# dask-contrib/dask-sql

Measured on NVIDIA H100. Metric: rows/s on Q3-shaped filter->join->groupby, higher is better.
Workload: dtype f64

## Files before the change

### dask-sql_b200/_lib.py

```python
import ctypes as C
import os

HERE = os.path.dirname(os.path.abspath(__file__))
LIB_PATH = os.environ.get("B200SQL_LIB") or os.path.join(HERE, "libb200sql.so")

I64, F64, U8 = 0, 1, 2
U32 = 3
COL_SENTINEL = 1
MAX_COLS, MAX_TERMS, MAX_AGGS, MAX_KEYS, MAX_GATHER, MAX_PROG = 16, 8, 8, 4, 8, 64
TILE = 4096
EQ, NE, LT, LE, GT, GE, IS_NULL, IS_NOT_NULL, IS_TRUE = range(9)
AGG_SUM, AGG_SUMF, AGG_MIN, AGG_MAX, AGG_COUNT, AGG_AND, AGG_OR, AGG_XOR = range(8)
JOIN_INNER, JOIN_LEFT, JOIN_SEMI, JOIN_ANTI = range(4)
EMPTY_KEY = -(1 << 63)

OP_LOAD, OP_CONST_I, OP_CONST_F, OP_CONST_NULL, OP_I2F, OP_F2I = 0, 1, 2, 3, 4, 5
OP_ADD_I, OP_SUB_I, OP_MUL_I, OP_DIV_I, OP_NEG_I, OP_ABS_I, OP_MOD_I = 10, 11, 12, 13, 14, 15, 16
OP_ADD_F, OP_SUB_F, OP_MUL_F, OP_DIV_F, OP_NEG_F, OP_ABS_F, OP_SQRT_F = 20, 21, 22, 23, 24, 25, 26
OP_EQ_I, OP_EQ_F = 30, 40
OP_AND, OP_OR, OP_NOT, OP_ISNULL_I, OP_ISNULL_F, OP_CASE, OP_FILLNA, OP_ORD2F = 50, 51, 52, 53, 54, 55, 56, 57
OP_DATEPART, OP_ADDMONTHS, OP_MAP = 60, 61, 62
OP_MATH_F, OP_MATH2_F, OP_POW_I = 63, 64, 65
(FN_CEIL, FN_FLOOR, FN_TRUNC, FN_ROUND, FN_SIGN, FN_DEGREES, FN_RADIANS, FN_EXP, FN_LN, FN_LOG10, FN_CBRT, FN_SIN,
 FN_COS, FN_TAN, FN_COT, FN_ASIN, FN_ACOS, FN_ATAN, FN_ATAN2, FN_POW, FN_MOD) = range(21)
# ... 149 lines not shown
    "b2_join_onepass": [C.POINTER(Scan), C.POINTER(C.c_int32), C.POINTER(JoinTable), C.c_int32, C.c_int32, _P, C.c_int32,
                        C.POINTER(C.c_int32), C.POINTER(_P), C.POINTER(_P), C.c_int32, C.POINTER(Col),
                        C.POINTER(C.c_int64), C.POINTER(_P), C.POINTER(_P), _P],
    "b2_join_agg": [C.POINTER(Scan), C.c_int32, C.POINTER(JoinTable), C.c_int32, C.POINTER(Col), C.POINTER(C.c_int64),
                    C.POINTER(JoinAgg), C.c_int32, _P, _P, C.c_int32, _P, _P],
    "b2_range_partition_hist": [C.POINTER(Scan), C.c_int32, C.c_int64, C.c_int64, C.c_int32, C.c_int32, _P, _P],
    "b2_range_partition_scan": [C.c_int32, _P, _P],
    "b2_range_partition_scatter": [C.POINTER(Scan), C.c_int32, C.c_int64, C.c_int64, C.c_int32, C.c_int32, C.c_int32,
                                   C.POINTER(C.c_int32), _P, C.POINTER(_P), _P, _P],
    "b2_range_partition": [C.POINTER(Scan), C.c_int32, C.c_int64, C.c_int64, C.c_int32, C.c_int32, C.c_int32,
                           C.POINTER(C.c_int32), _P, C.POINTER(_P), _P, _P],
    "b2_iota": [_P, C.c_int64, _P],
    "b2_bitwise_combine": [_P, _P, C.c_int64, C.c_int32, _P],
    "b2_peer_merge": [C.POINTER(PeerMerge), _P],
    "b2_sort_by": [C.POINTER(Col), C.c_int64, C.c_int32, C.c_int32, _P, _P, _P],
    "b2_dense_slots": [C.POINTER(Col), C.c_int64, C.c_int64, C.c_int32, _P, _P],
    "b2_star_build_dense": [C.POINTER(Col), _P, C.c_int64, _P, C.c_int64, C.c_int64, _P, _P, _P],
    "b2_star_build_mark": [C.POINTER(Scan), C.c_int32, C.c_int64, C.c_int64, _P, _P, _P],
    "b2_star_build_rank": [_P, C.c_int64, _P],
    "b2_star_build_fill": [C.POINTER(Scan), C.c_int32, C.c_int32, C.c_int64, C.c_int64, C.c_int64, C.c_int32, _P,
                           _P, _P],
    "b2_star_build_fill_packed": [C.POINTER(Scan), C.c_int32, C.c_int32, C.c_int64, C.c_int64, C.c_int64,
                                  C.c_int32, _P, _P, C.c_int32, _P],
    "b2_star_build_hash": [C.POINTER(Col), _P, C.c_int64, _P, _P, _P, C.c_int64, _P, _P],
    "b2_star_agg": [C.POINTER(Scan), C.c_int32, C.POINTER(StarLookup), C.POINTER(Agg), C.c_int32,
                    C.POINTER(AggState), _P],
    "b2_str_like": [_P, _P, C.c_int64, _P, C.c_int64, C.c_uint32, C.c_int32, _P, _P],
    "b2_str_lower_bound": [_P, _P, C.c_int64, _P, _P, C.c_int64, C.c_int32, _P, _P, _P],
}

EXPORTS = sorted(list(_SIGS) + ["b2_last_error", "b2_num_tiles", "b2_stats_ws_bytes", "b2_scan_agg_ws_bytes",
                                "b2_sort_ws_bytes", "b2_join_onepass_ws_bytes", "b2_range_partition_ws_bytes",
                                "b2_f64_to_ordered", "b2_ordered_to_f64"])


call_times = {} if os.environ.get("B200SQL_CALL_TIMES") == "1" else None


def _wrap(name):
    fn = getattr(_lib, name)
    fn.restype = C.c_int32
    fn.argtypes = _SIGS[name]

    if call_times is not None:
        import time

# ... 47 lines not shown
join_write_gather_keyed = _wrap("b2_join_write_gather_keyed")
join_key_layout = _wrap("b2_join_key_layout")
join_onepass = _wrap("b2_join_onepass")
join_onepass_ws_bytes = _lib.b2_join_onepass_ws_bytes
join_agg = _wrap("b2_join_agg")
range_partition = _wrap("b2_range_partition")
range_partition_hist = _wrap("b2_range_partition_hist")
range_partition_scan = _wrap("b2_range_partition_scan")
range_partition_scatter = _wrap("b2_range_partition_scatter")
range_partition_ws_bytes = _lib.b2_range_partition_ws_bytes
iota = _wrap("b2_iota")
bitwise_combine = _wrap("b2_bitwise_combine")
peer_merge = _wrap("b2_peer_merge")
sort_by = _wrap("b2_sort_by")
_lib.b2_sort_ws_bytes.restype = C.c_int64
_lib.b2_sort_ws_bytes.argtypes = [C.c_int64]
sort_ws_bytes = _lib.b2_sort_ws_bytes
dense_slots = _wrap("b2_dense_slots")
star_build_dense = _wrap("b2_star_build_dense")
star_build_mark = _wrap("b2_star_build_mark")
star_build_rank = _wrap("b2_star_build_rank")
star_build_fill = _wrap("b2_star_build_fill")
star_build_fill_packed = _wrap("b2_star_build_fill_packed")
star_build_hash = _wrap("b2_star_build_hash")
star_agg = _wrap("b2_star_agg")
str_like = _wrap("b2_str_like")
str_lower_bound = _wrap("b2_str_lower_bound")
num_tiles = _lib.b2_num_tiles
stats_ws_bytes = _lib.b2_stats_ws_bytes
scan_agg_ws_bytes = _lib.b2_scan_agg_ws_bytes
f64_to_ordered = _lib.b2_f64_to_ordered
ordered_to_f64 = _lib.b2_ordered_to_f64


def has_symbol(name):
    try:
        getattr(_lib, name)
        return True
    except AttributeError:
        return False
```

### dask-sql_b200/csrc/common.cuh

```cuda
#pragma once
#include <cuda_runtime.h>
#include <stdint.h>
#include <stdio.h>
#include <stdarg.h>
#include "b200sql.h"

#define B2_BLOCK 256
#define B2_WARPS (B2_BLOCK / 32)
#define FULL_MASK 0xffffffffu
#define B2_MAX_PARTIALS (132 * 16)

extern thread_local char g_b2_err[512];
static inline int32_t b2_fail(int32_t code, const char* fmt, ...) {
  va_list ap;
  va_start(ap, fmt);
  vsnprintf(g_b2_err, sizeof(g_b2_err), fmt, ap);
  va_end(ap);
  return code;
}
#define B2_CUDA_TRY(expr)                                                              \
  do {                                                                                 \
    cudaError_t e__ = (expr);                                                          \
    if (e__ != cudaSuccess)                                                            \
      return b2_fail(B2_ERR_CUDA, "%s failed: %s (%s:%d)", #expr, cudaGetErrorString(e__), \
// ... 73 lines not shown

__device__ __forceinline__ uint64_t b2_policy_stream() {
  uint64_t p;
  asm("createpolicy.fractional.L2::evict_first.b64 %0, 1.0;" : "=l"(p));
  return p;
}
__device__ __forceinline__ uint64_t b2_policy_keep() {
  uint64_t p;
  asm("createpolicy.fractional.L2::evict_last.b64 %0, 1.0;" : "=l"(p));
  return p;
}
__device__ __forceinline__ int64_t b2_ld_stream(const int64_t* p) {
  int64_t v;
  asm("ld.global.nc.L2::cache_hint.b64 %0, [%1], %2;" : "=l"(v) : "l"(p), "l"(b2_policy_stream()));
  return v;
}
__device__ __forceinline__ int32_t b2_ld_keep_i32(const int32_t* p) {
  int32_t v;
  asm("ld.global.nc.L2::cache_hint.b32 %0, [%1], %2;" : "=r"(v) : "l"(p), "l"(b2_policy_keep()));
  return v;
}
__device__ __forceinline__ void b2_st_stream(int64_t* p, int64_t v) {
  asm volatile("st.global.L2::cache_hint.b64 [%0], %1, %2;" ::"l"(p), "l"(v), "l"(b2_policy_stream()) : "memory");
}
__device__ __forceinline__ int64_t b2_ld_keep_i64(const int64_t* p) {
  int64_t v;
  asm("ld.global.nc.L2::cache_hint.b64 %0, [%1], %2;" : "=l"(v) : "l"(p), "l"(b2_policy_keep()));
  return v;
}
__device__ __forceinline__ int64_t b2_ld_cg_i64(const int64_t* p) {
  return __ldcg(reinterpret_cast<const long long*>(p));
}

__host__ __device__ __forceinline__ int64_t b2_ordered_from_bits(int64_t b) {
  return b ^ ((b >> 63) & 0x7fffffffffffffffLL);
}

__device__ __forceinline__ bool b2_cmp_i(int op, int64_t a, int64_t b) {
  switch (op) {
    case B2_EQ: return a == b;
    case B2_NE: return a != b;
    case B2_LT: return a < b;
    case B2_LE: return a <= b;
    case B2_GT: return a > b;
    default: return a >= b;
  }
// ... 329 lines not shown
```

### dask-sql_b200/csrc/groupby.cuh

```cuda
#pragma once
#include "common.cuh"
#include "pipeline.cuh"
#include "warpagg.cuh"

#define B2_GB_R 8
#define B2_GB_ROWS_PER_BLOCK (B2_BLOCK * B2_GB_R)
#define B2_MAX_PROBE 1024

template <int R, class LD>
__device__ __forceinline__ void b2_dense_slots_of(const b2_scan_t& s, const LD& ld, int key_col, int64_t kmin,
                                                  int64_t nslots, int64_t (&slot)[R]) {
  const b2_col_t& kc = s.cols[key_col];
  bool full;
  const uint32_t bits = b2_eval_terms<R>(s, ld, full);
  int64_t key[R];
  ld.template load<R>(key_col, bits, full, key);
  uint32_t kvalid = bits;
  if (kc.valid) kvalid = b2_valid_bits<R>(kc.valid, ld.row0, bits);
#pragma unroll
  for (int j = 0; j < R; ++j) {
    slot[j] = -1;
    if ((bits >> j) & 1) {
      if (!((kvalid >> j) & 1)) slot[j] = nslots - 1;
      else {
// ... 205 lines not shown
    out[i] = b2_is_null(key, i, raw) ? null_slot : (int32_t)(raw - kmin);
  }
}

__global__ void __launch_bounds__(B2_BLOCK)
b2_star_build_dense_kernel(const __grid_constant__ b2_col_t pk, const int32_t* __restrict__ sel, int64_t n_sel,
                           const int32_t* __restrict__ slot_of_row, int64_t kmin, int64_t range,
                           int32_t* __restrict__ lookup, int32_t* __restrict__ flags) {
  for (int64_t i = (int64_t)blockIdx.x * B2_BLOCK + threadIdx.x; i < n_sel; i += (int64_t)gridDim.x * B2_BLOCK) {
    const int64_t r = sel ? sel[i] : i;
    const int64_t raw = b2_load_raw(pk, r);
    if (b2_is_null(pk, r, raw)) continue;
    const uint64_t d = (uint64_t)raw - (uint64_t)kmin;
    if (d >= (uint64_t)range) continue;
    const int32_t old = atomicExch(lookup + d, slot_of_row[i]);
    if (old != -1) flags[0] = 1;
  }
}

__device__ __forceinline__ uint32_t b2_slot_word(uint32_t pos, int slot_bits) {
  return slot_bits == 16 ? pos >> 2 : __umulhi(pos, 0x55555556u);
}

template <bool FILL>
__global__ void __launch_bounds__(B2_BLOCK)
b2_star_build_scan_kernel(const __grid_constant__ b2_scan_t s, int pk_col, int grp_col, int64_t pk_min,
                          int64_t pk_range, int64_t grp_min, int32_t null_slot, uint64_t* __restrict__ dir,
                          void* __restrict__ slots, int slot_bits, int32_t* __restrict__ flags) {
  const int tile_off = (threadIdx.x >> 5) * (32 * B2_GB_R) + (threadIdx.x & 31);
  const b2_col_t& pc = s.cols[pk_col];
  const b2_col_t& gc = s.cols[grp_col];
  for (int64_t base = (int64_t)blockIdx.x * B2_GB_ROWS_PER_BLOCK; base < s.n;
       base += (int64_t)gridDim.x * B2_GB_ROWS_PER_BLOCK) {
    const b2_gld ld{&s, base + tile_off};
    bool full;
    const uint32_t bits = b2_eval_terms<B2_GB_R>(s, ld, full);
    int64_t pk[B2_GB_R];
    ld.template load<B2_GB_R>(pk_col, bits, full, pk);
    uint32_t live = bits;
    if (pc.valid) live &= b2_valid_bits<B2_GB_R>(pc.valid, ld.row0, bits);
#pragma unroll
    for (int j = 0; j < B2_GB_R; ++j) {
      const uint64_t d = (uint64_t)pk[j] - (uint64_t)pk_min;
      if (!(((live >> j) & 1) && d < (uint64_t)pk_range)) live &= ~(1u << j);
    }
    if (!FILL) {
#pragma unroll
      for (int j = 0; j < B2_GB_R; ++j) {
        if (!((live >> j) & 1)) continue;
        const uint64_t d = (uint64_t)pk[j] - (uint64_t)pk_min;
        const uint32_t b = 1u << (d & 31);
        if (atomicOr(reinterpret_cast<uint32_t*>(dir + (d >> 5)), b) & b) flags[0] = 1;
      }
    } else {
      int64_t grp[B2_GB_R];
      ld.template load<B2_GB_R>(grp_col, live, false, grp);
      uint32_t gnull = 0;
      if (gc.valid) gnull = live & ~b2_valid_bits<B2_GB_R>(gc.valid, ld.row0, live);
      uint32_t pos[B2_GB_R];
      int32_t v[B2_GB_R];
#pragma unroll
      for (int j = 0; j < B2_GB_R; ++j) {
        pos[j] = 0;
        v[j] = 0;
        if (!((live >> j) & 1)) continue;
        const uint64_t d = (uint64_t)pk[j] - (uint64_t)pk_min;
        const uint64_t w = dir[d >> 5];
        pos[j] = (uint32_t)(w >> 32) + __popc((uint32_t)w & ((1u << (d & 31)) - 1));
        v[j] = (gnull >> j) & 1 ? null_slot : (int32_t)(grp[j] - grp_min);
      }
      if (slot_bits == 32 || slot_bits == 16) {
#pragma unroll
        for (int j = 0; j < B2_GB_R; ++j) {
          if (!((live >> j) & 1)) continue;
          if (slot_bits == 32) static_cast<int32_t*>(slots)[pos[j]] = v[j];
          else static_cast<uint16_t*>(slots)[pos[j]] = (uint16_t)v[j];
        }
      } else {
        unsigned long long e[B2_GB_R], old[B2_GB_R];
        uint32_t q[B2_GB_R], sh[B2_GB_R];
#pragma unroll
        for (int j = 0; j < B2_GB_R; ++j) {
          q[j] = b2_slot_word(pos[j], 21);
          sh[j] = (pos[j] - q[j] * 3) * 21;
          e[j] = ((unsigned long long)(uint32_t)v[j] & 0x1FFFFFull) << sh[j];
          old[j] = 0;
        }
        unsigned long long* w = reinterpret_cast<unsigned long long*>(slots);
        for (uint32_t pend = live; pend;) {
          unsigned long long seen[B2_GB_R];
#pragma unroll
          for (int j = 0; j < B2_GB_R; ++j)
            if ((pend >> j) & 1) seen[j] = atomicCAS(w + q[j], old[j], (old[j] & ~(0x1FFFFFull << sh[j])) | e[j]);
#pragma unroll
          for (int j = 0; j < B2_GB_R; ++j) {
            if (!((pend >> j) & 1)) continue;
            if (seen[j] == old[j]) pend &= ~(1u << j);
            else old[j] = seen[j];
          }
        }
      }
    }
  }
}

#define B2_RANK_PER_THREAD 8
#define B2_RANK_TILE (B2_BLOCK * B2_RANK_PER_THREAD)

__device__ __forceinline__ uint32_t* b2_rank_half(uint64_t* dir, int64_t i) {
  return reinterpret_cast<uint32_t*>(dir + i) + 1;
}

template <bool WRITE>
__global__ void __launch_bounds__(B2_BLOCK) b2_star_rank_tile_kernel(uint64_t* __restrict__ dir, int64_t nwords) {
  __shared__ int warp_sums[B2_WARPS];
  __shared__ uint32_t tile_off;
  const int lane = threadIdx.x & 31, warp = threadIdx.x >> 5;
  const int64_t t0 = (int64_t)blockIdx.x * B2_RANK_TILE;
  const int64_t i0 = t0 + (int64_t)threadIdx.x * B2_RANK_PER_THREAD;
  if (WRITE && threadIdx.x == 0) tile_off = *b2_rank_half(dir, t0);
  uint32_t bits[B2_RANK_PER_THREAD];
  int tsum = 0;
#pragma unroll
  for (int k = 0; k < B2_RANK_PER_THREAD; ++k) {
    bits[k] = i0 + k < nwords ? (uint32_t)dir[i0 + k] : 0u;
    tsum += __popc(bits[k]);
  }
  int incl = tsum;
#pragma unroll
  for (int o = 1; o < 32; o <<= 1) {
    const int t = __shfl_up_sync(FULL_MASK, incl, o);
    if (lane >= o) incl += t;
  }
  if (lane == 31) warp_sums[warp] = incl;
  __syncthreads();
  if (!WRITE) {
    if (threadIdx.x == 0) {
      int total = 0;
      for (int w = 0; w < B2_WARPS; ++w) total += warp_sums[w];
      *b2_rank_half(dir, t0) = (uint32_t)total;
    }
    return;
  }
  uint32_t r = tile_off + (uint32_t)(incl - tsum);
  for (int w = 0; w < warp; ++w) r += (uint32_t)warp_sums[w];
#pragma unroll
  for (int k = 0; k < B2_RANK_PER_THREAD; ++k) {
    if (i0 + k < nwords) dir[i0 + k] = (uint64_t)bits[k] | ((uint64_t)r << 32);
    r += __popc(bits[k]);
  }
}

struct b2_scan_io_tile_off {
  uint64_t* dir;
  __device__ int64_t get(int64_t t) const { return *b2_rank_half(dir, t * B2_RANK_TILE); }
  __device__ void put(int64_t t, int64_t v) const { *b2_rank_half(dir, t * B2_RANK_TILE) = (uint32_t)v; }
};

__global__ void __launch_bounds__(B2_SCAN_THREADS) b2_star_rank_carry_kernel(uint64_t* __restrict__ dir, int64_t ntiles) {
  b2_block_exclusive_scan(b2_scan_io_tile_off{dir}, ntiles);
}

__global__ void __launch_bounds__(B2_BLOCK)
b2_star_build_hash_kernel(const __grid_constant__ b2_col_t pk, const int32_t* __restrict__ sel, int64_t n_sel,
                          const int32_t* __restrict__ slot_of_row, int64_t* __restrict__ tk,
                          int32_t* __restrict__ ts, int64_t cap, int32_t* __restrict__ flags) {
  for (int64_t i = (int64_t)blockIdx.x * B2_BLOCK + threadIdx.x; i < n_sel; i += (int64_t)gridDim.x * B2_BLOCK) {
    const int64_t r = sel ? sel[i] : i;
    const int64_t key = b2_load_raw(pk, r);
    if (b2_is_null(pk, r, key)) continue;
    if (key == B2_EMPTY_KEY) { flags[1] = 1; continue; }
    uint64_t h = b2_mix64((uint64_t)key) & (uint64_t)(cap - 1);
// ... 294 lines not shown

int32_t b2_dense_slots(const b2_col_t* key, int64_t n, int64_t kmin, int32_t null_slot, int32_t* out_slot,
                       void* stream) {
  B2_REQUIRE(key && out_slot, "null argument");
  if (n <= 0) return B2_OK;
  int grid = b2_wave_grid(b2_dense_slots_kernel, B2_BLOCK, (n + B2_BLOCK - 1) / B2_BLOCK);
  b2_dense_slots_kernel<<<grid, B2_BLOCK, 0, (cudaStream_t)stream>>>(*key, n, kmin, null_slot, out_slot);
  B2_CHECK_LAUNCH("b2_dense_slots_kernel");
  return B2_OK;
}

int32_t b2_star_build_dense(const b2_col_t* pk, const int32_t* sel, int64_t n_sel, const int32_t* slot_of_row,
                            int64_t kmin, int64_t range, int32_t* lookup, int32_t* d_flags, void* stream) {
  B2_REQUIRE(pk && slot_of_row && lookup && d_flags, "null argument");
  B2_REQUIRE(pk->dtype == B2_I64, "dense lookup needs an int64 key");
  if (n_sel <= 0) return B2_OK;
  int grid = b2_wave_grid(b2_star_build_dense_kernel, B2_BLOCK, (n_sel + B2_BLOCK - 1) / B2_BLOCK);
  b2_star_build_dense_kernel<<<grid, B2_BLOCK, 0, (cudaStream_t)stream>>>(*pk, sel, n_sel, slot_of_row, kmin,
                                                                           range, lookup, d_flags);
  B2_CHECK_LAUNCH("b2_star_build_dense_kernel");
  return B2_OK;
}

static int32_t b2_star_build_pass(bool fill, const b2_scan_t* scan, int32_t pk_col, int32_t grp_col,
                                  int64_t pk_min, int64_t pk_range, int64_t grp_min, int32_t null_slot,
                                  uint64_t* dir, void* slots, int32_t slot_bits, int32_t* d_flags, void* stream) {
  int32_t rc = b2_check_scan(scan);
  if (rc) return rc;
  B2_REQUIRE(pk_col >= 0 && pk_col < scan->ncols && grp_col >= 0 && grp_col < scan->ncols, "column out of range");
  B2_REQUIRE(scan->cols[pk_col].dtype == B2_I64 && scan->cols[grp_col].dtype == B2_I64, "dense keys must be int64");
  B2_REQUIRE(pk_range > 0 && pk_range < ((int64_t)1 << 31), "bad range");
  if (scan->n == 0) return B2_OK;
  int64_t nblk = (scan->n + B2_GB_ROWS_PER_BLOCK - 1) / B2_GB_ROWS_PER_BLOCK;
  if (fill) {
    int grid = b2_wave_grid(b2_star_build_scan_kernel<true>, B2_BLOCK, nblk);
    b2_star_build_scan_kernel<true><<<grid, B2_BLOCK, 0, (cudaStream_t)stream>>>(*scan, pk_col, grp_col, pk_min, pk_range,
                                                                                  grp_min, null_slot, dir, slots, slot_bits, d_flags);
  } else {
    int grid = b2_wave_grid(b2_star_build_scan_kernel<false>, B2_BLOCK, nblk);
    b2_star_build_scan_kernel<false><<<grid, B2_BLOCK, 0, (cudaStream_t)stream>>>(*scan, pk_col, grp_col, pk_min, pk_range,
                                                                                   grp_min, null_slot, dir, slots, slot_bits, d_flags);
  }
  B2_CHECK_LAUNCH("b2_star_build_scan_kernel");
  return B2_OK;
}

int32_t b2_star_build_mark(const b2_scan_t* scan, int32_t pk_col, int64_t pk_min, int64_t pk_range, uint64_t* dir,
                           int32_t* d_flags, void* stream) {
  B2_REQUIRE(dir && d_flags, "null argument");
  return b2_star_build_pass(false, scan, pk_col, pk_col, pk_min, pk_range, 0, 0, dir, nullptr, 32, d_flags, stream);
}

int32_t b2_star_build_rank(uint64_t* dir, int64_t pk_range, void* stream) {
  B2_REQUIRE(dir, "null argument");
  B2_REQUIRE(pk_range > 0 && pk_range < ((int64_t)1 << 31), "bad range");
  const int64_t nwords = (pk_range + 31) / 32;
  const int64_t ntiles = (nwords + B2_RANK_TILE - 1) / B2_RANK_TILE;
  b2_star_rank_tile_kernel<false><<<(unsigned)ntiles, B2_BLOCK, 0, (cudaStream_t)stream>>>(dir, nwords);
  B2_CHECK_LAUNCH("b2_star_rank_tile_kernel<false>");
  b2_star_rank_carry_kernel<<<1, B2_SCAN_THREADS, 0, (cudaStream_t)stream>>>(dir, ntiles);
  B2_CHECK_LAUNCH("b2_star_rank_carry_kernel");
  b2_star_rank_tile_kernel<true><<<(unsigned)ntiles, B2_BLOCK, 0, (cudaStream_t)stream>>>(dir, nwords);
  B2_CHECK_LAUNCH("b2_star_rank_tile_kernel<true>");
  return B2_OK;
}

int32_t b2_star_build_fill(const b2_scan_t* scan, int32_t pk_col, int32_t grp_col, int64_t pk_min,
                           int64_t pk_range, int64_t grp_min, int32_t null_slot, const uint64_t* dir,
                           int32_t* slots, void* stream) {
  return b2_star_build_fill_packed(scan, pk_col, grp_col, pk_min, pk_range, grp_min, null_slot, dir,
                                   reinterpret_cast<uint64_t*>(slots), 32, stream);
}

int32_t b2_star_build_fill_packed(const b2_scan_t* scan, int32_t pk_col, int32_t grp_col, int64_t pk_min,
                                  int64_t pk_range, int64_t grp_min, int32_t null_slot, const uint64_t* dir,
                                  uint64_t* slots, int32_t slot_bits, void* stream) {
  B2_REQUIRE(dir && slots, "null argument");
  B2_REQUIRE(slot_bits == 16 || slot_bits == 21 || slot_bits == 32, "slot_bits must be 16, 21 or 32");
  B2_REQUIRE(slot_bits == 32 || (null_slot >= 0 && null_slot < (1 << slot_bits)), "null_slot does not fit slot_bits");
  B2_REQUIRE(slot_bits == 32 || ((uintptr_t)slots & 7) == 0, "packed slots must be 8-byte aligned");
  return b2_star_build_pass(true, scan, pk_col, grp_col, pk_min, pk_range, grp_min, null_slot,
                            const_cast<uint64_t*>(dir), slots, slot_bits, nullptr, stream);
}

int32_t b2_star_build_hash(const b2_col_t* pk, const int32_t* sel, int64_t n_sel, const int32_t* slot_of_row,
                           int64_t* table_keys, int32_t* table_slots, int64_t cap, int32_t* d_flags,
                           void* stream) {
  B2_REQUIRE(pk && slot_of_row && table_keys && table_slots && d_flags, "null argument");
  B2_REQUIRE(pk->dtype == B2_I64, "star lookup needs an int64 key");
  B2_REQUIRE(b2_pow2(cap), "cap must be a power of two");
  if (n_sel <= 0) return B2_OK;
  int grid = b2_wave_grid(b2_star_build_hash_kernel, B2_BLOCK, (n_sel + B2_BLOCK - 1) / B2_BLOCK);
  b2_star_build_hash_kernel<<<grid, B2_BLOCK, 0, (cudaStream_t)stream>>>(*pk, sel, n_sel, slot_of_row, table_keys,
                                                                          table_slots, cap, d_flags);
  B2_CHECK_LAUNCH("b2_star_build_hash_kernel");
  return B2_OK;
}

int32_t b2_star_agg(const b2_scan_t* scan, int32_t fk_col, const b2_starlookup_t* lk, const b2_agg_t* aggs,
                    int32_t naggs, const b2_aggstate_t* st, void* stream) {
  int32_t rc = b2_check_scan(scan);
  if (rc) return rc;
  b2_aggs_arg aa;
  if ((rc = b2_check_aggs(scan, aggs, naggs, &aa))) return rc;
  if ((rc = b2_check_state(aa, st))) return rc;
// ... 30 lines not shown
```

### dask-sql_b200/executor.py

```python
import ctypes as C
import os
from collections import namedtuple
from typing import Dict, List, Optional, Sequence, Set

import numpy as np
import torch

from . import _lib as L
from . import device as D
from . import expr as E
from . import parallel as P
from . import strings as S
from .device import DeviceColumn, TermSpec, I64, F64, U8
from .expr import Expr, ColRef, Lit, Call
from .frame import LazyFrame, Source, TableSource, JoinSource, AggSource, SortSource, LimitSource
from .table import DeviceTable, HostColumn

DENSE_MAX_SLOTS = 1 << 27
_TORCH_DT = {I64: torch.int64, F64: torch.float64, U8: torch.uint8}

stats = {"launches": 0, "star_fused": 0, "dense_groupby": 0, "hash_groupby": 0, "dense_join": 0,
         "chain_join": 0, "keyed_join": 0, "partitioned_groupby": 0, "h2d_bytes": 0, "d2h_bytes": 0}


# ... 1482 lines not shown
            if part.n == 0:
                continue
            ctx = ScanCtx(part, q.dpred)
            pk_slot, g_slot = ctx.slot(q.pk_e), ctx.slot(q.ge)
            self._only_table_columns(ctx)
            self.dim_launch.append((ctx.scan(), pk_slot, g_slot))
            self.keep.append(ctx)
        self.fact_launch = []
        for part in fparts:
            if part.n == 0:
                continue
            ctx = ScanCtx(part, q.fpred)
            fk_slot = ctx.slot(q.fk_e)
            specs = [(ctx.slot(ka.expr), ka.op) for ka in q.plan.kaggs]
            self._only_table_columns(ctx)
            self.fact_launch.append((ctx.scan(), fk_slot, D.make_aggs(specs), len(specs), part.n))
            self.keep.append(ctx)
        self.slot_bits = _star_slot_bits(self.nslots - 1)
        slots_off, self.flags_off, words = _star_bitmap_words(q.prange, q.dn, self.slot_bits)
        self.lookup = torch.empty(words, dtype=torch.int32, device=dev)
        self.lk = lk = L.StarLookup()
        lk.dense, lk.dir, lk.kmin, lk.range, lk.slot_bits = 2, self.lookup.data_ptr(), q.pmin, q.prange, self.slot_bits
        lk.lookup = self.lookup.data_ptr() + 4 * slots_off
        self.tabs = [GroupState(dev, self.nslots, q.plan, need_present=True,
                                alloc=_padded_slots(self.nslots, q.sharded))]
        self.dirty = [False]
        self.peer = None
        self.epoch = 0
        self.free = [None, None]
        self.merge_bufs = {} if cached else None
        self.runs = 0

    def install_peer_merge(self, state):
        self.tabs, self.dirty, self.peer, self.arena, self.local_ready = state
        stats["peer_merge_plans"] = stats.get("peer_merge_plans", 0) + 1

    def build_peer_merge(self):
        rank, size = P.world()
        dev = self.dev
        alloc = _padded_slots(self.nslots, True)
        proto = self.tabs[0].table
        narr = sum(a is not None for a in proto.acc) + sum(c is not None for c in proto.cnt) + (proto.rows is not None)
        per_table = (narr * alloc * 8 + D.bitmap_words(alloc) * 4) + (narr + 2) * P.PeerArena.ALIGN
        arena = P.PeerArena(2 * per_table + 4 * P.PeerArena.ALIGN, dev)
        _, sig_off = arena.carve(L.MAX_PEERS, torch.int64, 0)
        chunk = alloc // size
# ... 61 lines not shown
            for name in needed:
                c = p[name]
                if not isinstance(c, DeviceColumn):
                    raise _NotPreparable()
                cols[name] = c
            parts.append(Part(cols, n))
        return parts

    def _only_table_columns(self, ctx: "ScanCtx"):
        if self.cached and any(not k.startswith("col:") for k in ctx.index):
            raise _NotPreparable()

    def run(self, src) -> Part:
        q = self.q
        i = self.runs & 1
        self.runs += 1
        buf = self.lookup
        main = D.cur_stream()
        sp = D.stream_ptr()
        if self.free[i] is not None:
            self.free[i].synchronize()
        if q.owner:
            with _Phase("build"):
                _star_bitmap_build(buf, self.dim_launch, q.pmin, q.prange, q.gmin, self.nslots - 1, q.dn,
                                   self.slot_bits, sp)
        if q.bcast:
            with _Phase("bcast"):
                P.broadcast_(buf, 0)
        ti = i if self.peer is not None else 0
        t = self.tabs[ti].table
        with _Phase("scan"):
            if self.dirty[ti]:
                t.reset()
            self.dirty[ti] = True
            for scan, fk_slot, aggs_arr, naggs, n in self.fact_launch:
                stats["launches"] += 1
                ev = _kernel_event_begin("b2_star_agg_kernel", n)
                L.star_agg(C.byref(scan), fk_slot, C.byref(self.lk), aggs_arr, naggs, C.byref(t.state), sp)
                _kernel_event_end(ev)
        if self.peer is not None:
            m, view = self.peer[ti]
            self.epoch += 1
            m.epoch = self.epoch
            with _Phase("peer_merge"):
                stats["launches"] += 1
                ev = _kernel_event_begin("b2_peer_merge_kernel", m.count)
                L.peer_merge(C.byref(m), sp)
                _kernel_event_end(ev)
# ... 9 lines not shown
                              key_nullable=q.gnull, check=buf[self.flags_off:], fallback=general)
        if self.cached:
            done = torch.cuda.Event()
            done.record(main)
            self.free[i] = done
        return out


class _NotPreparable(Exception):
    pass


def _star_slot_bits(null_slot):
    return 16 if null_slot < (1 << 16) else 21 if null_slot < (1 << 21) else 32


def _star_bitmap_words(prange, dn, slot_bits):
    slots = 2 * ((prange + 31) // 32)
    k = 64 // slot_bits
    flags = slots + 2 * ((min(dn, prange) + k - 1) // k)
    return slots, flags, flags + 4


def _star_bitmap_build(buf, launches, pmin, prange, gmin, null_slot, dn, slot_bits, sp):
    slots_off, flags_off, _ = _star_bitmap_words(prange, dn, slot_bits)
    base = buf.data_ptr()
    dirp, slots, flags = C.c_void_p(base), C.c_void_p(base + 4 * slots_off), C.c_void_p(base + 4 * flags_off)
    L.memset(dirp, 0, 4 * (flags_off if slot_bits < 32 else slots_off), sp)
    L.memset(flags, 0, 16, sp)
    for scan, pk_slot, _ in launches:
        stats["launches"] += 1
        L.star_build_mark(C.byref(scan), pk_slot, pmin, prange, dirp, flags, sp)
    stats["launches"] += 1
    L.star_build_rank(dirp, prange, sp)
    for scan, pk_slot, g_slot in launches:
        stats["launches"] += 1
        L.star_build_fill_packed(C.byref(scan), pk_slot, g_slot, pmin, prange, gmin, null_slot, dirp, slots,
                                 slot_bits, sp)


def _star_dense_fast(src, fact, dim, fk_e, pk_e, gexprs, aggs, fact_pred, dim_pred, sharded, dev) -> Optional[Part]:
    if len(gexprs) != 1 or not isinstance(dim.source, TableSource) or not isinstance(pk_e, ColRef):
        return None
    ge = E.substitute(gexprs[0], dim.exprs)
    if not isinstance(ge, ColRef) or ge.dtype != I64 or pk_e.dtype != I64:
        return None
    rank, world = P.world()
    dist = frame_distribution(dim)
    if world > 1 and dist == "sharded":
        return None
    table = dim.source.table
    owner = world == 1 or dist != "root" or rank == 0
    meta = None
    if owner:
        pst, gst = table.column_stats(pk_e.name), table.column_stats(ge.name)
        gnull = table.column_nullable(ge.name)
        meta = (pst.vmin, pst.vmax, gst.vmin, gst.vmax, table.nrows, gnull)
    if world > 1 and dist == "root":
        cache = table.__dict__.setdefault("_root_meta", {})
        ck = (pk_e.name, ge.name)
        if ck not in cache:
# ... 512 lines not shown
```

### include/b200sql.h

```cpp
#ifndef B200SQL_H
#define B200SQL_H
#include <stdint.h>
#ifdef __cplusplus
extern "C" {
#endif

#define B2_OK            0
#define B2_ERR_CUDA     -1
#define B2_ERR_ARG      -2

#define B2_I64 0
#define B2_F64 1
#define B2_U8  2
#define B2_U32 3

#define B2_MAX_COLS   16
#define B2_MAX_TERMS   8
#define B2_MAX_AGGS    8
#define B2_MAX_KEYS    4
#define B2_MAX_GATHER  8
#define B2_MAX_PROG   64
#define B2_TILE     4096

#define B2_EQ 0
// ... 320 lines not shown
                           int32_t nbuckets, int32_t ncarry, const int32_t* carry_cols, int64_t* out_key,
                           void* const* out_cols, void* d_ws, void* stream);

int64_t b2_sort_ws_bytes(int64_t n);
int32_t b2_iota(int32_t* out, int64_t n, void* stream);
int32_t b2_sort_by(const b2_col_t* col, int64_t n, int32_t descending, int32_t nulls_first, int32_t* idx,
                   void* ws, void* stream);

int32_t b2_dense_slots(const b2_col_t* key, int64_t n, int64_t kmin, int32_t null_slot,
                       int32_t* out_slot, void* stream);

int32_t b2_star_build_dense(const b2_col_t* pk, const int32_t* sel, int64_t n_sel,
                            const int32_t* slot_of_row, int64_t kmin, int64_t range,
                            int32_t* lookup, int32_t* d_flags, void* stream);
int32_t b2_star_build_mark(const b2_scan_t* scan, int32_t pk_col, int64_t pk_min, int64_t pk_range,
                           uint64_t* dir, int32_t* d_flags, void* stream);
int32_t b2_star_build_rank(uint64_t* dir, int64_t pk_range, void* stream);
int32_t b2_star_build_fill(const b2_scan_t* scan, int32_t pk_col, int32_t grp_col, int64_t pk_min,
                           int64_t pk_range, int64_t grp_min, int32_t null_slot, const uint64_t* dir,
                           int32_t* slots, void* stream);
int32_t b2_star_build_fill_packed(const b2_scan_t* scan, int32_t pk_col, int32_t grp_col, int64_t pk_min,
                                  int64_t pk_range, int64_t grp_min, int32_t null_slot, const uint64_t* dir,
                                  uint64_t* slots, int32_t slot_bits, void* stream);
int32_t b2_star_build_hash(const b2_col_t* pk, const int32_t* sel, int64_t n_sel,
                           const int32_t* slot_of_row, int64_t* table_keys, int32_t* table_slots,
                           int64_t cap, int32_t* d_flags, void* stream);

typedef struct b2_starlookup {
  int32_t dense;
  int32_t slot_bits;
  const int32_t* lookup;
  int64_t kmin;
  int64_t range;
  const int64_t* table_keys;
  const int32_t* table_slots;
  int64_t cap;
  const uint64_t* dir;
} b2_starlookup_t;

int32_t b2_star_agg(const b2_scan_t* scan, int32_t fk_col, const b2_starlookup_t* lk,
                    const b2_agg_t* aggs, int32_t naggs, const b2_aggstate_t* st, void* stream);

#ifdef __cplusplus
}
#endif
#endif
// ... 1 lines not shown
```

Measured before the change: 81.22 billion.

## Replace mark/fill dimension scans with a staged array packed during rank

```diff
diff --git a/dask-sql_b200/_lib.py b/dask-sql_b200/_lib.py
--- a/dask-sql_b200/_lib.py
+++ b/dask-sql_b200/_lib.py
@@ -195,6 +195,9 @@
                            _P, _P],
     "b2_star_build_fill_packed": [C.POINTER(Scan), C.c_int32, C.c_int32, C.c_int64, C.c_int64, C.c_int64,
                                   C.c_int32, _P, _P, C.c_int32, _P],
+    "b2_star_build_stage": [C.POINTER(Scan), C.c_int32, C.c_int32, C.c_int64, C.c_int64, C.c_int64, C.c_int32,
+                            _P, _P, _P],
+    "b2_star_build_rank_pack": [_P, C.c_int64, _P, _P, _P, C.c_int32, _P, _P],
     "b2_star_build_hash": [C.POINTER(Col), _P, C.c_int64, _P, _P, _P, C.c_int64, _P, _P],
     "b2_star_agg": [C.POINTER(Scan), C.c_int32, C.POINTER(StarLookup), C.POINTER(Agg), C.c_int32,
                     C.POINTER(AggState), _P],
@@ -288,6 +291,8 @@
 star_build_rank = _wrap("b2_star_build_rank")
 star_build_fill = _wrap("b2_star_build_fill")
 star_build_fill_packed = _wrap("b2_star_build_fill_packed")
+star_build_stage = _wrap("b2_star_build_stage")
+star_build_rank_pack = _wrap("b2_star_build_rank_pack")
 star_build_hash = _wrap("b2_star_build_hash")
 star_agg = _wrap("b2_star_agg")
 str_like = _wrap("b2_str_like")
diff --git a/dask-sql_b200/csrc/common.cuh b/dask-sql_b200/csrc/common.cuh
--- a/dask-sql_b200/csrc/common.cuh
+++ b/dask-sql_b200/csrc/common.cuh
@@ -119,6 +119,9 @@
 }
 __device__ __forceinline__ void b2_st_stream(int64_t* p, int64_t v) {
   asm volatile("st.global.L2::cache_hint.b64 [%0], %1, %2;" ::"l"(p), "l"(v), "l"(b2_policy_stream()) : "memory");
+}
+__device__ __forceinline__ void b2_st_keep_i32(int32_t* p, int32_t v) {
+  asm volatile("st.global.L2::cache_hint.b32 [%0], %1, %2;" ::"l"(p), "r"(v), "l"(b2_policy_keep()) : "memory");
 }
 __device__ __forceinline__ int64_t b2_ld_keep_i64(const int64_t* p) {
   int64_t v;
diff --git a/dask-sql_b200/csrc/groupby.cuh b/dask-sql_b200/csrc/groupby.cuh
--- a/dask-sql_b200/csrc/groupby.cuh
+++ b/dask-sql_b200/csrc/groupby.cuh
@@ -251,11 +251,18 @@
   return slot_bits == 16 ? pos >> 2 : __umulhi(pos, 0x55555556u);
 }
 
-template <bool FILL>
+enum { B2_STAR_MARK, B2_STAR_FILL, B2_STAR_STAGE };
+
+template <int PASS>
 __global__ void __launch_bounds__(B2_BLOCK)
 b2_star_build_scan_kernel(const __grid_constant__ b2_scan_t s, int pk_col, int grp_col, int64_t pk_min,
                           int64_t pk_range, int64_t grp_min, int32_t null_slot, uint64_t* __restrict__ dir,
-                          void* __restrict__ slots, int slot_bits, int32_t* __restrict__ flags) {
+                          void* __restrict__ slots, int slot_bits, int32_t* __restrict__ flags,
+                          unsigned long long* __restrict__ count) {
+  constexpr bool FILL = PASS != B2_STAR_MARK;
+  __shared__ unsigned long long cta_live;
+  if (PASS == B2_STAR_STAGE && threadIdx.x == 0) cta_live = 0;
+  uint32_t nlive = 0;
   const int tile_off = (threadIdx.x >> 5) * (32 * B2_GB_R) + (threadIdx.x & 31);
   const b2_col_t& pc = s.cols[pk_col];
   const b2_col_t& gc = s.cols[grp_col];
@@ -293,12 +300,22 @@
         pos[j] = 0;
         v[j] = 0;
         if (!((live >> j) & 1)) continue;
-        const uint64_t d = (uint64_t)pk[j] - (uint64_t)pk_min;
-        const uint64_t w = dir[d >> 5];
-        pos[j] = (uint32_t)(w >> 32) + __popc((uint32_t)w & ((1u << (d & 31)) - 1));
+        if (PASS == B2_STAR_FILL) {
+          const uint64_t d = (uint64_t)pk[j] - (uint64_t)pk_min;
+          const uint64_t w = dir[d >> 5];
+          pos[j] = (uint32_t)(w >> 32) + __popc((uint32_t)w & ((1u << (d & 31)) - 1));
+        }
         v[j] = (gnull >> j) & 1 ? null_slot : (int32_t)(grp[j] - grp_min);
       }
-      if (slot_bits == 32 || slot_bits == 16) {
+      if (PASS == B2_STAR_STAGE) {
+        nlive += __popc(live);
+#pragma unroll
+        for (int j = 0; j < B2_GB_R; ++j) {
+          if (!((live >> j) & 1)) continue;
+          const uint64_t d = (uint64_t)pk[j] - (uint64_t)pk_min;
+          b2_st_keep_i32(static_cast<int32_t*>(slots) + d, v[j]);
+        }
+      } else if (slot_bits == 32 || slot_bits == 16) {
 #pragma unroll
         for (int j = 0; j < B2_GB_R; ++j) {
           if (!((live >> j) & 1)) continue;
@@ -331,6 +348,13 @@
       }
     }
   }
+  if (PASS == B2_STAR_STAGE) {
+    __syncthreads();
+    const uint32_t n = __reduce_add_sync(FULL_MASK, nlive);
+    if ((threadIdx.x & 31) == 0 && n) atomicAdd(&cta_live, (unsigned long long)n);
+    __syncthreads();
+    if (threadIdx.x == 0 && cta_live) atomicAdd(count, cta_live);
+  }
 }
 
 #define B2_RANK_PER_THREAD 8
@@ -340,8 +364,111 @@
   return reinterpret_cast<uint32_t*>(dir + i) + 1;
 }
 
-template <bool WRITE>
-__global__ void __launch_bounds__(B2_BLOCK) b2_star_rank_tile_kernel(uint64_t* __restrict__ dir, int64_t nwords) {
+struct b2_star_pack_t {
+  const int32_t* stage;
+  uint64_t* slots;
+  int slot_bits;
+  unsigned long long* count;
+  int32_t* flags;
+  int64_t nkeys;
+};
+
+#define B2_STAGE_EMPTY (-1)
+
+__device__ __forceinline__ void b2_star_stage_bits(const b2_star_pack_t& pa, int64_t w0,
+                                                   uint32_t (&bits)[B2_RANK_PER_THREAD]) {
+  const int lane = threadIdx.x & 31;
+  for (int s = 0; s < 32; ++s) {
+    const int64_t key0 = (w0 + s * B2_RANK_PER_THREAD) * 32 + lane;
+    int32_t e[B2_RANK_PER_THREAD];
+#pragma unroll
+    for (int j = 0; j < B2_RANK_PER_THREAD; ++j)
+      e[j] = key0 + j * 32 < pa.nkeys ? __ldcg(pa.stage + key0 + j * 32) : B2_STAGE_EMPTY;
+#pragma unroll
+    for (int j = 0; j < B2_RANK_PER_THREAD; ++j) {
+      const uint32_t m = __ballot_sync(FULL_MASK, e[j] != B2_STAGE_EMPTY);
+      if (lane == s) bits[j] = m;
+    }
+  }
+}
+
+__device__ __forceinline__ void b2_slot_put(uint64_t* slots, uint32_t pos, uint32_t v, int slot_bits) {
+  if (slot_bits == 32) {
+    reinterpret_cast<int32_t*>(slots)[pos] = (int32_t)v;
+  } else if (slot_bits == 16) {
+    reinterpret_cast<uint16_t*>(slots)[pos] = (uint16_t)v;
+  } else {
+    const uint32_t q = b2_slot_word(pos, 21);
+    atomicOr(reinterpret_cast<unsigned long long*>(slots + q),
+             (unsigned long long)(v & 0x1FFFFFu) << ((pos - q * 3) * 21));
+  }
+}
+
+#define B2_PACK_BUF (32 * B2_RANK_PER_THREAD + 4)
+
+__device__ __forceinline__ void b2_star_pack_warp(const b2_star_pack_t& pa, const uint32_t (&bits)[B2_RANK_PER_THREAD],
+                                                  uint32_t r0, uint32_t r1, int64_t w0) {
+  __shared__ uint32_t buf_all[B2_WARPS][B2_PACK_BUF];
+  uint32_t* buf = buf_all[threadIdx.x >> 5];
+  const int lane = threadIdx.x & 31;
+  const uint32_t below = (1u << lane) - 1;
+  const int bw = pa.slot_bits, k = 64 / bw;
+  const uint32_t mask = bw == 32 ? 0xFFFFFFFFu : (1u << bw) - 1;
+  const uint32_t p_begin = __shfl_sync(FULL_MASK, r0, 0), p_end = __shfl_sync(FULL_MASK, r1, 31);
+  if (p_begin == p_end) return;
+  uint32_t q0 = p_begin / k;
+  int n = (int)(p_begin - q0 * k);
+  if (lane < n) buf[lane] = 0;
+  for (int s = 0; s < 32; ++s) {
+    const int64_t key0 = (w0 + s * B2_RANK_PER_THREAD) * 32 + lane;
+    uint32_t b[B2_RANK_PER_THREAD];
+    int32_t v[B2_RANK_PER_THREAD];
+#pragma unroll
+    for (int j = 0; j < B2_RANK_PER_THREAD; ++j) {
+      b[j] = __shfl_sync(FULL_MASK, bits[j], s);
+      v[j] = (b[j] >> lane) & 1 ? __ldcs(pa.stage + key0 + j * 32) : 0;
+    }
+    uint32_t any = 0;
+#pragma unroll
+    for (int j = 0; j < B2_RANK_PER_THREAD; ++j) any |= b[j];
+    if (any) {
+      int off = n;
+#pragma unroll
+      for (int j = 0; j < B2_RANK_PER_THREAD; ++j) {
+        if ((b[j] >> lane) & 1) buf[off + __popc(b[j] & below)] = (uint32_t)v[j];
+        off += __popc(b[j]);
+      }
+      __syncwarp();
+      const int nw = off / k;
+      for (int q = lane; q < nw; q += 32) {
+        const uint32_t* e = buf + q * k;
+        const uint32_t p0 = (q0 + q) * k;
+        if (p0 >= p_begin) {
+          uint64_t word = 0;
+#pragma unroll
+          for (int f = 0; f < 4; ++f)
+            if (f < k) word |= (uint64_t)(e[f] & mask) << (f * bw);
+          pa.slots[q0 + q] = word;
+        } else {
+          for (int f = 0; f < k; ++f)
+            if (p0 + f >= p_begin) b2_slot_put(pa.slots, p0 + f, e[f], bw);
+        }
+      }
+      const int rest = off - nw * k;
+      const uint32_t t = lane < rest ? buf[nw * k + lane] : 0u;
+      __syncwarp();
+      if (lane < rest) buf[lane] = t;
+      __syncwarp();
+      n = rest;
+      q0 += nw;
+    }
+  }
+  if (lane < n && q0 * k + lane >= p_begin) b2_slot_put(pa.slots, q0 * k + lane, buf[lane], bw);
+}
+
+template <bool WRITE, bool PACK = false>
+__global__ void __launch_bounds__(B2_BLOCK) b2_star_rank_tile_kernel(uint64_t* __restrict__ dir, int64_t nwords,
+                                                                      const __grid_constant__ b2_star_pack_t pa) {
   __shared__ int warp_sums[B2_WARPS];
   __shared__ uint32_t tile_off;
   const int lane = threadIdx.x & 31, warp = threadIdx.x >> 5;
@@ -350,10 +477,19 @@
   if (WRITE && threadIdx.x == 0) tile_off = *b2_rank_half(dir, t0);
   uint32_t bits[B2_RANK_PER_THREAD];
   int tsum = 0;
-#pragma unroll
-  for (int k = 0; k < B2_RANK_PER_THREAD; ++k) {
-    bits[k] = i0 + k < nwords ? (uint32_t)dir[i0 + k] : 0u;
-    tsum += __popc(bits[k]);
+  if (PACK && !WRITE) {
+    b2_star_stage_bits(pa, t0 + (int64_t)warp * 32 * B2_RANK_PER_THREAD, bits);
+#pragma unroll
+    for (int k = 0; k < B2_RANK_PER_THREAD; ++k) {
+      if (i0 + k < nwords) dir[i0 + k] = bits[k];
+      tsum += __popc(bits[k]);
+    }
+  } else {
+#pragma unroll
+    for (int k = 0; k < B2_RANK_PER_THREAD; ++k) {
+      bits[k] = i0 + k < nwords ? (uint32_t)dir[i0 + k] : 0u;
+      tsum += __popc(bits[k]);
+    }
   }
   int incl = tsum;
 #pragma unroll
@@ -373,10 +509,18 @@
   }
   uint32_t r = tile_off + (uint32_t)(incl - tsum);
   for (int w = 0; w < warp; ++w) r += (uint32_t)warp_sums[w];
+  const uint32_t r0 = r;
 #pragma unroll
   for (int k = 0; k < B2_RANK_PER_THREAD; ++k) {
     if (i0 + k < nwords) dir[i0 + k] = (uint64_t)bits[k] | ((uint64_t)r << 32);
     r += __popc(bits[k]);
+  }
+  if (PACK) {
+    b2_star_pack_warp(pa, bits, r0, r, t0 + (int64_t)warp * 32 * B2_RANK_PER_THREAD);
+    if (i0 <= nwords - 1 && nwords - 1 < i0 + B2_RANK_PER_THREAD) {
+      if (*pa.count != (unsigned long long)r) pa.flags[0] = 1;
+      *pa.count = 0;
+    }
   }
 }
 
@@ -717,9 +861,10 @@
   return B2_OK;
 }
 
-static int32_t b2_star_build_pass(bool fill, const b2_scan_t* scan, int32_t pk_col, int32_t grp_col,
+static int32_t b2_star_build_pass(int pass, const b2_scan_t* scan, int32_t pk_col, int32_t grp_col,
                                   int64_t pk_min, int64_t pk_range, int64_t grp_min, int32_t null_slot,
-                                  uint64_t* dir, void* slots, int32_t slot_bits, int32_t* d_flags, void* stream) {
+                                  uint64_t* dir, void* slots, int32_t slot_bits, int32_t* d_flags,
+                                  unsigned long long* count, void* stream) {
   int32_t rc = b2_check_scan(scan);
   if (rc) return rc;
   B2_REQUIRE(pk_col >= 0 && pk_col < scan->ncols && grp_col >= 0 && grp_col < scan->ncols, "column out of range");
@@ -727,15 +872,14 @@
   B2_REQUIRE(pk_range > 0 && pk_range < ((int64_t)1 << 31), "bad range");
   if (scan->n == 0) return B2_OK;
   int64_t nblk = (scan->n + B2_GB_ROWS_PER_BLOCK - 1) / B2_GB_ROWS_PER_BLOCK;
-  if (fill) {
-    int grid = b2_wave_grid(b2_star_build_scan_kernel<true>, B2_BLOCK, nblk);
-    b2_star_build_scan_kernel<true><<<grid, B2_BLOCK, 0, (cudaStream_t)stream>>>(*scan, pk_col, grp_col, pk_min, pk_range,
-                                                                                  grp_min, null_slot, dir, slots, slot_bits, d_flags);
-  } else {
-    int grid = b2_wave_grid(b2_star_build_scan_kernel<false>, B2_BLOCK, nblk);
-    b2_star_build_scan_kernel<false><<<grid, B2_BLOCK, 0, (cudaStream_t)stream>>>(*scan, pk_col, grp_col, pk_min, pk_range,
-                                                                                   grp_min, null_slot, dir, slots, slot_bits, d_flags);
-  }
+  auto launch = [&](auto kernel) {
+    int grid = b2_wave_grid(kernel, B2_BLOCK, nblk);
+    kernel<<<grid, B2_BLOCK, 0, (cudaStream_t)stream>>>(*scan, pk_col, grp_col, pk_min, pk_range, grp_min, null_slot,
+                                                        dir, slots, slot_bits, d_flags, count);
+  };
+  if (pass == B2_STAR_FILL) launch(b2_star_build_scan_kernel<B2_STAR_FILL>);
+  else if (pass == B2_STAR_STAGE) launch(b2_star_build_scan_kernel<B2_STAR_STAGE>);
+  else launch(b2_star_build_scan_kernel<B2_STAR_MARK>);
   B2_CHECK_LAUNCH("b2_star_build_scan_kernel");
   return B2_OK;
 }
@@ -743,21 +887,56 @@
 int32_t b2_star_build_mark(const b2_scan_t* scan, int32_t pk_col, int64_t pk_min, int64_t pk_range, uint64_t* dir,
                            int32_t* d_flags, void* stream) {
   B2_REQUIRE(dir && d_flags, "null argument");
-  return b2_star_build_pass(false, scan, pk_col, pk_col, pk_min, pk_range, 0, 0, dir, nullptr, 32, d_flags, stream);
-}
-
-int32_t b2_star_build_rank(uint64_t* dir, int64_t pk_range, void* stream) {
+  return b2_star_build_pass(B2_STAR_MARK, scan, pk_col, pk_col, pk_min, pk_range, 0, 0, dir, nullptr, 32, d_flags,
+                            nullptr, stream);
+}
+
+int32_t b2_star_build_stage(const b2_scan_t* scan, int32_t pk_col, int32_t grp_col, int64_t pk_min,
+                            int64_t pk_range, int64_t grp_min, int32_t null_slot, int32_t* stage, uint64_t* d_count,
+                            void* stream) {
+  B2_REQUIRE(stage && d_count, "null argument");
+  B2_REQUIRE(null_slot >= 0, "null_slot must be >= 0");
+  return b2_star_build_pass(B2_STAR_STAGE, scan, pk_col, grp_col, pk_min, pk_range, grp_min, null_slot, nullptr,
+                            stage, 32, nullptr, reinterpret_cast<unsigned long long*>(d_count), stream);
+}
+
+static int32_t b2_star_rank_launch(uint64_t* dir, int64_t pk_range, const b2_star_pack_t* pack, void* stream) {
   B2_REQUIRE(dir, "null argument");
   B2_REQUIRE(pk_range > 0 && pk_range < ((int64_t)1 << 31), "bad range");
   const int64_t nwords = (pk_range + 31) / 32;
   const int64_t ntiles = (nwords + B2_RANK_TILE - 1) / B2_RANK_TILE;
-  b2_star_rank_tile_kernel<false><<<(unsigned)ntiles, B2_BLOCK, 0, (cudaStream_t)stream>>>(dir, nwords);
-  B2_CHECK_LAUNCH("b2_star_rank_tile_kernel<false>");
+  const b2_star_pack_t none{};
+  if (pack) {
+    b2_star_rank_tile_kernel<false, true><<<(unsigned)ntiles, B2_BLOCK, 0, (cudaStream_t)stream>>>(dir, nwords, *pack);
+    B2_CHECK_LAUNCH("b2_star_rank_tile_kernel<false, true>");
+  } else {
+    b2_star_rank_tile_kernel<false><<<(unsigned)ntiles, B2_BLOCK, 0, (cudaStream_t)stream>>>(dir, nwords, none);
+    B2_CHECK_LAUNCH("b2_star_rank_tile_kernel<false>");
+  }
   b2_star_rank_carry_kernel<<<1, B2_SCAN_THREADS, 0, (cudaStream_t)stream>>>(dir, ntiles);
   B2_CHECK_LAUNCH("b2_star_rank_carry_kernel");
-  b2_star_rank_tile_kernel<true><<<(unsigned)ntiles, B2_BLOCK, 0, (cudaStream_t)stream>>>(dir, nwords);
-  B2_CHECK_LAUNCH("b2_star_rank_tile_kernel<true>");
-  return B2_OK;
+  if (pack) {
+    b2_star_rank_tile_kernel<true, true><<<(unsigned)ntiles, B2_BLOCK, 0, (cudaStream_t)stream>>>(dir, nwords, *pack);
+    B2_CHECK_LAUNCH("b2_star_rank_tile_kernel<true, true>");
+  } else {
+    b2_star_rank_tile_kernel<true><<<(unsigned)ntiles, B2_BLOCK, 0, (cudaStream_t)stream>>>(dir, nwords, none);
+    B2_CHECK_LAUNCH("b2_star_rank_tile_kernel<true>");
+  }
+  return B2_OK;
+}
+
+int32_t b2_star_build_rank(uint64_t* dir, int64_t pk_range, void* stream) {
+  return b2_star_rank_launch(dir, pk_range, nullptr, stream);
+}
+
+int32_t b2_star_build_rank_pack(uint64_t* dir, int64_t pk_range, const int32_t* stage, uint64_t* d_count,
+                                uint64_t* slots, int32_t slot_bits, int32_t* d_flags, void* stream) {
+  B2_REQUIRE(stage && d_count && slots && d_flags, "null argument");
+  B2_REQUIRE(slot_bits == 16 || slot_bits == 21 || slot_bits == 32, "slot_bits must be 16, 21 or 32");
+  B2_REQUIRE(((uintptr_t)slots & 7) == 0, "slots must be 8-byte aligned");
+  const b2_star_pack_t pack{stage, slots, slot_bits, reinterpret_cast<unsigned long long*>(d_count), d_flags,
+                            pk_range};
+  return b2_star_rank_launch(dir, pk_range, &pack, stream);
 }
 
 int32_t b2_star_build_fill(const b2_scan_t* scan, int32_t pk_col, int32_t grp_col, int64_t pk_min,
@@ -774,8 +953,8 @@
   B2_REQUIRE(slot_bits == 16 || slot_bits == 21 || slot_bits == 32, "slot_bits must be 16, 21 or 32");
   B2_REQUIRE(slot_bits == 32 || (null_slot >= 0 && null_slot < (1 << slot_bits)), "null_slot does not fit slot_bits");
   B2_REQUIRE(slot_bits == 32 || ((uintptr_t)slots & 7) == 0, "packed slots must be 8-byte aligned");
-  return b2_star_build_pass(true, scan, pk_col, grp_col, pk_min, pk_range, grp_min, null_slot,
-                            const_cast<uint64_t*>(dir), slots, slot_bits, nullptr, stream);
+  return b2_star_build_pass(B2_STAR_FILL, scan, pk_col, grp_col, pk_min, pk_range, grp_min, null_slot,
+                            const_cast<uint64_t*>(dir), slots, slot_bits, nullptr, nullptr, stream);
 }
 
 int32_t b2_star_build_hash(const b2_col_t* pk, const int32_t* sel, int64_t n_sel, const int32_t* slot_of_row,
diff --git a/dask-sql_b200/executor.py b/dask-sql_b200/executor.py
--- a/dask-sql_b200/executor.py
+++ b/dask-sql_b200/executor.py
@@ -1528,6 +1528,9 @@
         self.lk = lk = L.StarLookup()
         lk.dense, lk.dir, lk.kmin, lk.range, lk.slot_bits = 2, self.lookup.data_ptr(), q.pmin, q.prange, self.slot_bits
         lk.lookup = self.lookup.data_ptr() + 4 * slots_off
+        if q.owner:
+            self.stage = torch.empty(q.prange, dtype=torch.int32, device=dev)
+            self.stage_count = torch.zeros(1, dtype=torch.int64, device=dev)
         self.tabs = [GroupState(dev, self.nslots, q.plan, need_present=True,
                                 alloc=_padded_slots(self.nslots, q.sharded))]
         self.dirty = [False]
@@ -1635,8 +1638,8 @@
             self.free[i].synchronize()
         if q.owner:
             with _Phase("build"):
-                _star_bitmap_build(buf, self.dim_launch, q.pmin, q.prange, q.gmin, self.nslots - 1, q.dn,
-                                   self.slot_bits, sp)
+                _star_bitmap_build(buf, self.stage, self.stage_count, self.dim_launch, q.pmin, q.prange, q.gmin,
+                                   self.nslots - 1, q.dn, self.slot_bits, sp)
         if q.bcast:
             with _Phase("bcast"):
                 P.broadcast_(buf, 0)
@@ -1692,21 +1695,20 @@
     return slots, flags, flags + 4
 
 
-def _star_bitmap_build(buf, launches, pmin, prange, gmin, null_slot, dn, slot_bits, sp):
+def _star_bitmap_build(buf, stage, count, launches, pmin, prange, gmin, null_slot, dn, slot_bits, sp):
     slots_off, flags_off, _ = _star_bitmap_words(prange, dn, slot_bits)
     base = buf.data_ptr()
     dirp, slots, flags = C.c_void_p(base), C.c_void_p(base + 4 * slots_off), C.c_void_p(base + 4 * flags_off)
-    L.memset(dirp, 0, 4 * (flags_off if slot_bits < 32 else slots_off), sp)
+    if slot_bits == 21:
+        L.memset(slots, 0, 4 * (flags_off - slots_off), sp)
     L.memset(flags, 0, 16, sp)
-    for scan, pk_slot, _ in launches:
-        stats["launches"] += 1
-        L.star_build_mark(C.byref(scan), pk_slot, pmin, prange, dirp, flags, sp)
-    stats["launches"] += 1
-    L.star_build_rank(dirp, prange, sp)
+    stagep, countp = C.c_void_p(stage.data_ptr()), C.c_void_p(count.data_ptr())
+    L.memset(stagep, 0xFF, 4 * prange, sp)
     for scan, pk_slot, g_slot in launches:
         stats["launches"] += 1
-        L.star_build_fill_packed(C.byref(scan), pk_slot, g_slot, pmin, prange, gmin, null_slot, dirp, slots,
-                                 slot_bits, sp)
+        L.star_build_stage(C.byref(scan), pk_slot, g_slot, pmin, prange, gmin, null_slot, stagep, countp, sp)
+    stats["launches"] += 1
+    L.star_build_rank_pack(dirp, prange, stagep, countp, slots, slot_bits, flags, sp)
 
 
 def _star_dense_fast(src, fact, dim, fk_e, pk_e, gexprs, aggs, fact_pred, dim_pred, sharded, dev) -> Optional[Part]:
diff --git a/include/b200sql.h b/include/b200sql.h
--- a/include/b200sql.h
+++ b/include/b200sql.h
@@ -366,6 +366,11 @@
 int32_t b2_star_build_fill_packed(const b2_scan_t* scan, int32_t pk_col, int32_t grp_col, int64_t pk_min,
                                   int64_t pk_range, int64_t grp_min, int32_t null_slot, const uint64_t* dir,
                                   uint64_t* slots, int32_t slot_bits, void* stream);
+int32_t b2_star_build_stage(const b2_scan_t* scan, int32_t pk_col, int32_t grp_col, int64_t pk_min,
+                            int64_t pk_range, int64_t grp_min, int32_t null_slot, int32_t* stage,
+                            uint64_t* d_count, void* stream);
+int32_t b2_star_build_rank_pack(uint64_t* dir, int64_t pk_range, const int32_t* stage, uint64_t* d_count,
+                                uint64_t* slots, int32_t slot_bits, int32_t* d_flags, void* stream);
 int32_t b2_star_build_hash(const b2_col_t* pk, const int32_t* sel, int64_t n_sel,
                            const int32_t* slot_of_row, int64_t* table_keys, int32_t* table_slots,
                            int64_t cap, int32_t* d_flags, void* stream);
```

Measured after the change: 82.62 billion (median of 6 runs). 1.7% higher.
